# fanzhongyi/ExploreMultiModal

Hardware: AMD Instinct MI355X
Metric: image-text pairs/sec fwd+bwd, VLMo-Base, 1/2/4/8 MI355X; % bf16 MFMA roofline (higher is better)
Workload: dtype bf16

## Files before the change

exploremultimodal_amd/csrc/block.hip:

```cpp
#include "common.h"
#include "vlmo_hip.h"
#include <algorithm>
#include <map>
#include <vector>

namespace {
constexpr int GELU_DERIV = 4;


struct Events {
    std::vector<hipEvent_t> pool;
    hipEvent_t get(size_t i) {
        while (pool.size() <= i) {
            hipEvent_t e = nullptr;
            (void)hipEventCreateWithFlags(&e, hipEventDisableTiming);
            pool.push_back(e);
        }
        return pool[i];
    }
};
Events& events() {
    static thread_local std::map<int, Events> per_device;
    int dev = 0;
    (void)hipGetDevice(&dev);
// ... 288 lines not shown
    VLMO_CHECK_ARG(!two || nsets > batch || nb <= nsets,
                   "vlmo_stack_bwd: %d temporary sets cannot cover deferred batches of %d blocks", nsets, batch);
    Events& ev = events();
    Deferred D;
    D.store = s->wgrad_store != 0;
    std::vector<int> batch_of(nb, -1);
    int n_batches = 0, waited_upto = -1;
    auto flush = [&]() -> int {
        if (D.blocks.empty()) return 0;
        if (two) {
            hipEvent_t f = ev.get(2 * n_batches);
            (void)hipEventRecord(f, st);
            (void)hipStreamWaitEvent(side, f, 0);
        }
        std::stable_sort(D.tn.begin(), D.tn.end(), [](const VlmoTnProblem& a, const VlmoTnProblem& b) { return a.M > b.M; });
        TRY(vlmo_gemm_tn_multi(VLMO_BF16, D.tn.data(), (int)D.tn.size(), side));
        TRY(vlmo_colwork_multi(VLMO_BF16, D.col.data(), (int)D.col.size(), side));
        if (two) (void)hipEventRecord(ev.get(2 * n_batches + 1), side);
        if (s->grad_ready)
            for (int i : D.blocks)
                if (s->grad_ready[i]) (void)hipEventRecord((hipEvent_t)s->grad_ready[i], side);
        ++n_batches;
        D.tn.clear();
        D.col.clear();
        D.blocks.clear();
        return 0;
    };
    auto set_free = [&](int kk) -> int {
        if (!two || kk < nsets || kk >= nb) return 0;
        int need = batch_of[kk - nsets];
        if (need < 0 || need >= n_batches) {
            TRY(flush());
// ... 41 lines not shown
```

exploremultimodal_amd/csrc/elementwise.hip:

```cpp
#include "common.h"
#include "vlmo_hip.h"
#include <stdarg.h>
#include <stdio.h>

static thread_local char g_err[512] = "";
void vlmo_set_error(const char* fmt, ...) {
    va_list ap;
    va_start(ap, fmt);
    vsnprintf(g_err, sizeof(g_err), fmt, ap);
    va_end(ap);
}
extern "C" const char* vlmo_last_error(void) { return g_err; }
extern "C" int vlmo_abi_version(void) { return VLMO_ABI_VERSION; }

namespace {

__device__ __forceinline__ float fold_column(const float* __restrict__ ws, int ld, int ncols, int c, int r0, int r1) {
    float a = 0.f;
    if (c < ncols)
        for (int r = r0 + threadIdx.y; r < r1; r += 4) a += ws[(size_t)r * ld + c];
    return a;
}
template <typename T>
__device__ __forceinline__ void colsum8(const T* __restrict__ x, int ld, int ncols, int c8, int r0, int r1, float (&acc)[8]) {
    typedef typename Elem<T>::v8 v8;
#pragma unroll
    for (int j = 0; j < 8; ++j) acc[j] = 0.f;
    if (c8 < ncols) {
        for (int mb = r0 + threadIdx.y; mb < r1; mb += 16) {
            v8 v[4];
#pragma unroll
            for (int k = 0; k < 4; ++k) {
                const int m = mb + 4 * k;
                v[k] = *(const v8*)(x + (size_t)(m < r1 ? m : mb) * ld + c8);
            }
#pragma unroll
            for (int k = 0; k < 4; ++k)
                if (mb + 4 * k < r1)
#pragma unroll
                    for (int j = 0; j < 8; ++j) acc[j] += (float)v[k][j];
        }
    }
}

__global__ __launch_bounds__(256) void reduce_partials_kernel(const float* __restrict__ ws, int nblk, int ncols,
                                                              float* __restrict__ out0, int n0,
                                                              float* __restrict__ out1, int rows_per_slice,
                                                              float* __restrict__ out2, float* __restrict__ out3) {
    __shared__ float red[4][64];
    const int c = blockIdx.x * 64 + threadIdx.x;
    const int r0 = blockIdx.y * rows_per_slice, r1 = min(nblk, r0 + rows_per_slice);
    red[threadIdx.y][threadIdx.x] = fold_column(ws, ncols, ncols, c, r0, r1);
    __syncthreads();
    if (threadIdx.y == 0 && c < ncols) {
        const float t = red[0][threadIdx.x] + red[1][threadIdx.x] + red[2][threadIdx.x] + red[3][threadIdx.x];
        const int k = c / n0;
        float* base = k == 0 ? out0 : (k == 1 ? out1 : (k == 2 ? out2 : out3));
        if (base) atomicAdd(base + (c - k * n0), t);
    }
}

template <typename T> __device__ __forceinline__ f32x4 ld4(const T* p);
template <> __device__ __forceinline__ f32x4 ld4<bf16>(const bf16* p) {
    const bf16x4 v = *(const bf16x4*)p;
    return f32x4{(float)v[0], (float)v[1], (float)v[2], (float)v[3]};
}
template <> __device__ __forceinline__ f32x4 ld4<f16>(const f16* p) {
// ... 56 lines not shown
            ag += *(const f32x4*)(red + (y * 2 + 0) * d + c4);
            ab += *(const f32x4*)(red + (y * 2 + 1) * d + c4);
        }
        *(f32x4*)(ws + (size_t)blockIdx.x * 2 * d + c4) = ag;
        *(f32x4*)(ws + (size_t)blockIdx.x * 2 * d + d + c4) = ab;
    }
}

template <typename T>
__global__ __launch_bounds__(256) void colsum_kernel(const T* __restrict__ x, int ld, float* __restrict__ ws, int M,
                                                     int N, int rows_per_block) {
    __shared__ float red[4][64][8];
    const int c8 = (blockIdx.x * 64 + threadIdx.x) * 8;
    float acc[8];
    const int r0 = blockIdx.y * rows_per_block, r1 = min(M, r0 + rows_per_block);
    colsum8(x, ld, N, c8, r0, r1, acc);
#pragma unroll
    for (int j = 0; j < 8; ++j) red[threadIdx.y][threadIdx.x][j] = acc[j];
    __syncthreads();
    if (threadIdx.y == 0 && c8 < N) {
#pragma unroll
        for (int j = 0; j < 8; ++j)
            ws[(size_t)blockIdx.y * N + c8 + j] = red[0][threadIdx.x][j] + red[1][threadIdx.x][j] +
                                                  red[2][threadIdx.x][j] + red[3][threadIdx.x][j];
    }
}

constexpr int MAX_COL_JOBS = 32;
struct ColMulti {
    int n;
    int b0[MAX_COL_JOBS + 1];
    int gx[MAX_COL_JOBS], rps[MAX_COL_JOBS];
    VlmoColJob j[MAX_COL_JOBS];
};
template <typename T>
__global__ __launch_bounds__(256) void colwork_multi_kernel(const ColMulti cm) {
    __shared__ float red[4][64][8];
    int ji = 0;
#pragma unroll
    for (int q = 1; q < MAX_COL_JOBS; ++q)
        if (q < cm.n && (int)blockIdx.x >= cm.b0[q]) ji = q;
    ji = __builtin_amdgcn_readfirstlane(ji);
    const VlmoColJob& J = cm.j[ji];
    const int local = blockIdx.x - cm.b0[ji], gx = cm.gx[ji], rps = cm.rps[ji];
    const int bx = local % gx, by = local / gx;
    const int r0 = by * rps, r1 = min(J.rows, r0 + rps);
    const int tx = threadIdx.x, ty = threadIdx.y;
    if (J.kind == 0) {
        const int c = bx * 64 + tx;
        red[ty][tx][0] = fold_column((const float*)J.src, J.ld, J.ncols, c, r0, r1);
        __syncthreads();
        if (ty == 0 && c < J.ncols) {
            const float t = red[0][tx][0] + red[1][tx][0] + red[2][tx][0] + red[3][tx][0];
            const int k = c / J.n0;
            float* base = J.out[k];
            if (base) atomicAdd(base + (c - k * J.n0), t);
        }
    } else {
        const int c8 = (bx * 64 + tx) * 8;
        float acc[8];
        colsum8((const T*)J.src, J.ld, J.ncols, c8, r0, r1, acc);
#pragma unroll
        for (int jj = 0; jj < 8; ++jj) red[ty][tx][jj] = acc[jj];
        __syncthreads();
        if (ty == 0 && c8 < J.ncols) {
#pragma unroll
            for (int jj = 0; jj < 8; ++jj) {
                const int c = c8 + jj;
                const int k = c / J.n0;
                float* base = J.out[k];
                if (base) atomicAdd(base + (c - k * J.n0), red[0][tx][jj] + red[1][tx][jj] + red[2][tx][jj] + red[3][tx][jj]);
            }
        }
    }
}

template <typename T>
__global__ __launch_bounds__(256) void cast_weight_kernel(const float* __restrict__ src, int rows, int cols,
                                                          T* __restrict__ dst, T* __restrict__ dstT) {
    __shared__ float tile[32][33];
    const int c0 = blockIdx.x * 32, r0 = blockIdx.y * 32;
#pragma unroll
    for (int k = 0; k < 4; ++k) {
        const int r = r0 + threadIdx.y + 8 * k, c = c0 + threadIdx.x;
        float v = 0.f;
        if (r < rows && c < cols) {
            v = src[(size_t)r * cols + c];
            if (dst) dst[(size_t)r * cols + c] = (T)v;
        }
// ... 350 lines not shown
    for (int c = threadIdx.x; c < d; c += 256) {
        const int idx = embed_txt_red_index(c);
#pragma unroll
        for (int w = 0; w < 4; ++w) row[w * d + c] = red[0][w][idx] + red[1][w][idx] + red[2][w][idx] + red[3][w][idx];
    }
}

__global__ __launch_bounds__(256) void embed_txt_fold_kernel(const float* __restrict__ ws, int nrows, int maxlen, int d,
                                                             float* __restrict__ dln_w, float* __restrict__ dln_b,
                                                             float* __restrict__ dtype0, float* __restrict__ dbtype0,
                                                             float* __restrict__ dpos) {
    __shared__ float red[4][4][64];
    const int c = blockIdx.x * 64 + threadIdx.x, ld = 4 * d;
    if (blockIdx.y == 0) {
#pragma unroll
        for (int w = 0; w < 4; ++w) red[w][threadIdx.y][threadIdx.x] = fold_column(ws + w * d, ld, d, c, 0, nrows);
        __syncthreads();
        if (c < d) {
            const int w = threadIdx.y;
            float* out = w == 0 ? dln_w : (w == 1 ? dln_b : (w == 2 ? dtype0 : dbtype0));
            if (out) out[c] += red[w][0][threadIdx.x] + red[w][1][threadIdx.x] + red[w][2][threadIdx.x] + red[w][3][threadIdx.x];
        }
    } else {
        const int t = blockIdx.y - 1;
        red[0][threadIdx.y][threadIdx.x] = fold_column(ws + (size_t)t * ld + 3 * d, maxlen * ld, d, c, 0, nrows / maxlen);
        __syncthreads();
        if (threadIdx.y == 0 && c < d && dpos)
            dpos[(size_t)t * d + c] += red[0][0][threadIdx.x] + red[0][1][threadIdx.x] + red[0][2][threadIdx.x] + red[0][3][threadIdx.x];
    }
}

}

int fold_partials(const VlmoColJob& job, VlmoColJob* fold, hipStream_t stream) {
    if (fold) {
        *fold = job;
        return 0;
    }
    int slices = job.rows >= 64 ? 8 : 1;
    const int rps = (job.rows + slices - 1) / slices;
// ... 58 lines not shown
    if (dtype == VLMO_BF16)
        hipLaunchKernelGGL(colsum_kernel<bf16>, grid, block, 0, stream, (const bf16*)x, ld, ws, M, N, rpb);
    else if (dtype == VLMO_F16)
        hipLaunchKernelGGL(colsum_kernel<f16>, grid, block, 0, stream, (const f16*)x, ld, ws, M, N, rpb);
    else {
        vlmo_set_error("vlmo_colsum: dtype must be bf16 or f16");
        return -1;
    }
    VLMO_CHECK_LAUNCH("vlmo_colsum");
    return fold_partials(fold_job(ws, N, grid.y, N, N, out), nullptr, stream);
}

extern "C" int vlmo_colwork_multi(int dtype, const VlmoColJob* jobs, int n, hipStream_t stream) {
    VLMO_CHECK_ARG(jobs && n >= 1, "vlmo_colwork_multi: no jobs");
    VLMO_CHECK_ARG(dtype == VLMO_BF16 || dtype == VLMO_F16, "vlmo_colwork_multi: dtype must be bf16 or f16");
    for (int q0 = 0; q0 < n; q0 += MAX_COL_JOBS) {
        const int nq = n - q0 < MAX_COL_JOBS ? n - q0 : MAX_COL_JOBS;
        ColMulti cm{};
        cm.n = nq;
        int b = 0;
        for (int q = 0; q < nq; ++q) {
            const VlmoColJob& J = jobs[q0 + q];
            VLMO_CHECK_ARG(J.src && J.rows > 0 && J.ncols > 0 && J.n0 > 0 && J.ncols <= 4 * J.n0 && J.ld >= J.ncols,
                           "vlmo_colwork_multi: bad job %d", q0 + q);
            VLMO_CHECK_ARG(J.kind == 0 || (J.kind == 1 && J.ncols % 8 == 0 && J.ld % 8 == 0),
                           "vlmo_colwork_multi: job %d: matrix column sums need ncols, ld multiples of 8", q0 + q);
            cm.j[q] = J;
            cm.gx[q] = J.kind == 0 ? (J.ncols + 63) / 64 : (J.ncols / 8 + 63) / 64;
            int slices = J.kind == 0 ? (J.rows >= 64 ? 8 : 1) : (J.rows >= 2048 ? 32 : (J.rows >= 256 ? 8 : 1));
            int rps = (J.rows + slices - 1) / slices;
            if (J.kind == 1) rps = ((rps + 15) / 16) * 16;
            slices = (J.rows + rps - 1) / rps;
            cm.rps[q] = rps;
            cm.b0[q] = b;
            b += cm.gx[q] * slices;
        }
        for (int q = nq; q <= MAX_COL_JOBS; ++q) cm.b0[q] = b;
        if (dtype == VLMO_F16)
            hipLaunchKernelGGL(colwork_multi_kernel<f16>, dim3(b), dim3(64, 4), 0, stream, cm);
        else
            hipLaunchKernelGGL(colwork_multi_kernel<bf16>, dim3(b), dim3(64, 4), 0, stream, cm);
        VLMO_CHECK_LAUNCH("vlmo_colwork_multi");
    }
    return 0;
}

extern "C" int vlmo_cast_weight(int dtype, const float* src, int rows, int cols, void* dst, void* dstT,
                                hipStream_t stream) {
    VLMO_CHECK_ARG(src && (dst || dstT), "vlmo_cast_weight: null pointer");
    VLMO_CHECK_ARG(rows > 0 && cols > 0, "vlmo_cast_weight: empty matrix");
    dim3 grid((cols + 31) / 32, (rows + 31) / 32), block(32, 8);
    if (dtype == VLMO_BF16)
// ... 151 lines not shown
```

exploremultimodal_amd/csrc/gemm_tn.hip:

```cpp
#include "gemm_common.h"
#include "tn_multi_plan.h"

namespace {

struct GemmTN {
    const void* A;
    const void* B;
    float* C;
    int M, N1, N2, lda, ldb, ldc;
    int kt_per_split, tiles;
    float alpha;
    float* slab;
    int mode;
};

__device__ __attribute__((aligned(256))) char tn_zero_page[256];

__device__ __forceinline__ int tn_swz(int row) { return ((row & 3) << 2) | ((row >> 2) & 3); }

template <typename T, int BM, int BN, int WM, int WN, bool PP = false>
__device__ __forceinline__ void gemm_tn_body(const GemmTN& p, const int lid) {
    typedef typename Elem<T>::v8 v8;
    typedef typename Elem<T>::v4 v4;
    constexpr int NW = WM * WN;
// ... 227 lines not shown
                        atomicAdd(c, p.alpha * acc[i][j][r]);
                }
            }
        }
}

template <typename T, int BM, int BN, int WM, int WN, bool PP = false>
__global__ __launch_bounds__(WM * WN * 64, 2) void gemm_tn_kernel(const GemmTN p) {
    gemm_tn_body<T, BM, BN, WM, WN, PP>(p, xcd_remap(blockIdx.x, gridDim.x));
}
constexpr int TN_LDS_256 = 2 * 4 * 64 * 256;

struct GemmTNMulti {
    GemmTN p[MAX_TN_PROBS];
    uint16_t order[MAX_TN_ORDER];
};
template <typename T>
__global__ __launch_bounds__(512, 2) void gemm_tn_multi_kernel(const GemmTNMulti mp) {
    const uint32_t code = mp.order[blockIdx.x];
    if (code == TN_NOP) return;
    int gi = (int)(code >> 12);
    const int lid_in = __builtin_amdgcn_readfirstlane((int)(code & 0xFFFu));
    gi = __builtin_amdgcn_readfirstlane(gi);
    const GemmTN& q = mp.p[gi];
    GemmTN p;
    p.A = uniform_ptr(q.A), p.B = uniform_ptr(q.B), p.C = (float*)uniform_ptr(q.C);
    p.M = __builtin_amdgcn_readfirstlane(q.M), p.N1 = __builtin_amdgcn_readfirstlane(q.N1);
    p.N2 = __builtin_amdgcn_readfirstlane(q.N2), p.lda = __builtin_amdgcn_readfirstlane(q.lda);
    p.ldb = __builtin_amdgcn_readfirstlane(q.ldb), p.ldc = __builtin_amdgcn_readfirstlane(q.ldc);
    p.kt_per_split = __builtin_amdgcn_readfirstlane(q.kt_per_split), p.tiles = __builtin_amdgcn_readfirstlane(q.tiles);
    p.alpha = __builtin_bit_cast(float, __builtin_amdgcn_readfirstlane(__builtin_bit_cast(int, q.alpha)));
    p.slab = nullptr;
    p.mode = __builtin_amdgcn_readfirstlane(q.mode);
// ... 79 lines not shown
        if (dtype == VLMO_F16)
            hipLaunchKernelGGL((gemm_tn_kernel<f16, 128, 128, 2, 2>), grid, dim3(256), 65536, stream, p);
        else
            hipLaunchKernelGGL((gemm_tn_kernel<bf16, 128, 128, 2, 2>), grid, dim3(256), 65536, stream, p);
    }
    VLMO_CHECK_LAUNCH("vlmo_gemm_tn");
    if (use_slab) {
        const long total = (long)N1 * (N2 / 4);
        const int rg = (int)((total + 255) / 256 < 2048 ? (total + 255) / 256 : 2048);
        hipLaunchKernelGGL(tn_reduce_kernel, dim3(rg), dim3(256), 0, stream, ws, pl.splits, N1, N2, C, ldc, alpha);
        VLMO_CHECK_LAUNCH("vlmo_gemm_tn(reduce)");
    }
    return 0;
}

extern "C" int vlmo_gemm_tn_multi(int dtype, const VlmoTnProblem* probs, int n, hipStream_t stream) {
    VLMO_CHECK_ARG(probs && n >= 1, "vlmo_gemm_tn_multi: no problems");
    VLMO_CHECK_ARG(dtype == VLMO_BF16 || dtype == VLMO_F16, "vlmo_gemm_tn_multi: dtype must be bf16 or f16");
    for (int q = 0; q < n; ++q) {
        const VlmoTnProblem& r = probs[q];
        VLMO_CHECK_ARG(r.A && r.B && r.C, "vlmo_gemm_tn_multi: null operand in problem %d", q);
        VLMO_CHECK_ARG(r.M > 0 && r.N1 >= 8 && r.N2 >= 8 && r.N1 % 8 == 0 && r.N2 % 8 == 0 && r.lda % 8 == 0 &&
                           r.ldb % 8 == 0 && r.lda >= r.N1 && r.ldb >= r.N2 && r.ldc >= r.N2,
                       "vlmo_gemm_tn_multi: bad shape in problem %d (M=%d N1=%d N2=%d)", q, r.M, r.N1, r.N2);
    }
    const TnMultiPlan plan = plan_tn_multi(probs, n);
    VLMO_CHECK_ARG(plan.error.empty(), "%s", plan.error.c_str());
    static DeviceOnce attr;
    if (attr.first()) {
        (void)hipFuncSetAttribute((const void*)gemm_tn_multi_kernel<bf16>, hipFuncAttributeMaxDynamicSharedMemorySize, TN_LDS_256);
        (void)hipFuncSetAttribute((const void*)gemm_tn_multi_kernel<f16>, hipFuncAttributeMaxDynamicSharedMemorySize, TN_LDS_256);
    }
    for (const TnLaunchPlan& L : plan.launches) {
        GemmTNMulti mp{};
        double flops = 0;
        for (int q = 0; q < L.nq; ++q) {
            const VlmoTnProblem& r = probs[L.q0 + q];
            const VlmoTnProblemPlan& s = L.p[q];
            if (s.zero_first) {
                hipError_t rc = hipMemset2DAsync(r.C, (size_t)r.ldc * 4, 0, (size_t)r.N2 * 4, r.N1, stream);
                if (rc != hipSuccess) {
                    vlmo_set_error("vlmo_gemm_tn_multi: memset failed: %s", hipGetErrorString(rc));
                    return (int)rc;
                }
            }
            mp.p[q] = GemmTN{r.A, r.B, r.C, r.M, r.N1, r.N2, r.lda, r.ldb, r.ldc, s.kt_per_split, s.tiles, r.alpha, nullptr, s.mode};
            flops += 2.0 * r.M * r.N1 * r.N2;
        }
        std::copy(L.order, L.order + L.grid, mp.order);
        ProfScope prof(73, flops, stream);
        if (dtype == VLMO_F16)
            hipLaunchKernelGGL((gemm_tn_multi_kernel<f16>), dim3(L.grid), dim3(512), TN_LDS_256, stream, mp);
        else
            hipLaunchKernelGGL((gemm_tn_multi_kernel<bf16>), dim3(L.grid), dim3(512), TN_LDS_256, stream, mp);
        VLMO_CHECK_LAUNCH("vlmo_gemm_tn_multi");
    }
    return 0;
}

extern "C" int vlmo_gemm_tn_multi_plan(const VlmoTnProblem* probs, int n, int32_t* n_launches, int32_t* launch_q0,
                                       VlmoTnProblemPlan* prob, int32_t* grid, uint16_t* order) {
    VLMO_CHECK_ARG(probs && n >= 1, "vlmo_gemm_tn_multi: no problems");
    VLMO_CHECK_ARG(n_launches && launch_q0 && prob && grid && order, "vlmo_gemm_tn_multi_plan: null output");
    const TnMultiPlan plan = plan_tn_multi(probs, n);
    VLMO_CHECK_ARG(plan.error.empty(), "%s", plan.error.c_str());
    *n_launches = (int32_t)plan.launches.size();
    for (size_t k = 0; k < plan.launches.size(); ++k) {
        const TnLaunchPlan& L = plan.launches[k];
        launch_q0[k] = L.q0, launch_q0[k + 1] = L.q0 + L.nq;
        std::copy(L.p, L.p + L.nq, prob + L.q0);
        grid[k] = L.grid;
        std::copy(L.order, L.order + L.grid, order + k * MAX_TN_ORDER);
    }
    return 0;
}
```

exploremultimodal_amd/csrc/tn_multi_plan.h:

```cpp
#pragma once
#include "vlmo_hip.h"
#include <algorithm>
#include <cstdio>
#include <string>
#include <vector>

constexpr int MAX_TN_PROBS = 16;
constexpr int MAX_TN_ORDER = 1024;
constexpr uint16_t TN_NOP = 0xFFFF;
enum { TN_ATOMIC = 0, TN_ACCUM = 1, TN_STORE = 2 };

struct TnLaunchPlan {
    int q0, nq;
    VlmoTnProblemPlan p[MAX_TN_PROBS];
    int grid;
    uint16_t order[MAX_TN_ORDER];
};
struct TnMultiPlan {
    std::vector<TnLaunchPlan> launches;
    std::string error;
};

inline int64_t tn_tiles256(const VlmoTnProblem& r) { return (((int64_t)r.N1 + 255) / 256) * (((int64_t)r.N2 + 255) / 256); }
inline int tn_ktiles(const VlmoTnProblem& r) { return (int)(((int64_t)r.M + 63) / 64); }
// ... 47 lines not shown
            for (int x = 0; x < 8; ++x)
                for (size_t k = i + cnt * x / 8; k < i + cnt * (x + 1) / 8; ++k) bins[x].push_back(jobs[k].code);
        }
        size_t deepest = 0;
        for (int x = 0; x < 8; ++x) deepest = std::max(deepest, bins[x].size());
        if (deepest * 8 > (size_t)MAX_TN_ORDER)
            return fail("vlmo_gemm_tn_multi: %zu workgroups exceed one launch (pass fewer problems per call)", jobs.size());
        L.grid = (int)deepest * 8;
        for (int b = 0; b < L.grid; ++b) {
            const std::vector<uint16_t>& bin = bins[b & 7];
            L.order[b] = (size_t)(b >> 3) < bin.size() ? bin[b >> 3] : TN_NOP;
        }
    }
    return plan;
}
```

exploremultimodal_amd/hip.py:

```python
import ctypes
import os

import numpy as np
import torch

_HERE = os.path.dirname(os.path.abspath(__file__))
LIB_PATH = os.environ.get('VLMO_HIP_LIB') or os.path.join(_HERE, 'lib', 'libvlmo_hip.so')

BF16, F16, F32 = 0, 1, 2
EPI_BIAS, EPI_BIAS_GELU, EPI_RESID, EPI_DGELU, EPI_F32, EPI_DUAL, EPI_ARGMAX, EPI_CE, EPI_CE_BWD = 0, 1, 2, 3, 4, 5, 6, 7, 8

_vp, _i32, _u32, _u64, _f32, _i64 = (ctypes.c_void_p, ctypes.c_int32, ctypes.c_uint32,
                                     ctypes.c_uint64, ctypes.c_float, ctypes.c_int64)


class Epilogue(ctypes.Structure):
    _fields_ = [('out', _vp), ('out2', _vp), ('bias', _vp), ('gamma', _vp),
                ('resid', _vp), ('row_scale', _vp), ('row_index', _vp), ('aux', _vp),
                ('ldo', _i32), ('ld2', _i32), ('relu', _i32),
                ('drop_thresh', _u32), ('inv_keep', _f32), ('beta', _f32),
                ('seed', _u64), ('colpart', _vp)]


_fp = _vp
# ... 87 lines not shown
    'vlmo_argmax_reduce': [_vp, _i32, _vp, _i32, _vp],
    'vlmo_dvae_embed': [_vp, _vp, _vp, _vp, _i32, _i32, _i32, _vp],
    'vlmo_upsample2_nhwc': [_vp, _vp, _i32, _i32, _i32, _i32, _vp],
    'vlmo_dvae_out_head': [_vp, _vp, _vp, _vp, _i32, _i32, _i32, _i32, _i32, _vp],
    'vlmo_conv4s2_nhwc': [_i32, _vp, _i32, _i32, _i32, _i32, _vp, _i32, _vp, ctypes.POINTER(Epilogue), _vp],
    'vlmo_convt4s2_nhwc': [_i32, _vp, _i32, _i32, _i32, _i32, _vp, _i32, _vp, ctypes.POINTER(Epilogue), _vp],
    'vlmo_dvae_patch4s2': [_vp, _vp, _i32, _i32, _i32, _i32, _i32, _vp],
    'vlmo_dvae_out_head_linear': [_vp, _vp, _vp, _vp, _i32, _i32, _i32, _i32, _i32, _vp],
    'vlmo_ce_reduce': [_vp, _i32, _vp, _i32, _vp, _vp, _vp, _i32, _vp],
    'vlmo_stack_fwd': [ctypes.POINTER(StackDesc), _vp],
    'vlmo_stack_bwd': [ctypes.POINTER(StackDesc), _vp],
    'vlmo_gemm_tn_multi': [_i32, ctypes.POINTER(TnProblem), _i32, _vp],
    'vlmo_gemm_tn_multi_plan': [ctypes.POINTER(TnProblem), _i32, ctypes.POINTER(_i32), ctypes.POINTER(_i32),
                                ctypes.POINTER(TnProblemPlan), ctypes.POINTER(_i32), ctypes.POINTER(ctypes.c_uint16)],
    'vlmo_colwork_multi': [_i32, ctypes.POINTER(ColJob), _i32, _vp],
    'vlmo_event_create': [ctypes.POINTER(ctypes.c_void_p)],
    'vlmo_event_destroy': [_vp],
    'vlmo_stream_wait_event': [_vp, _vp],
    'vlmo_profile_start': [_i32],
    'vlmo_gemm_nt_grouped': [_i32, _i32, _i32, _i32, _vp, _i32, _vp, _i32, _vp, _i32, _i32, _vp, _vp],
    'vlmo_mt_grad_norm': [ctypes.c_void_p, _f32, _f32, _vp, _vp, _vp],
    'vlmo_mt_adam': [ctypes.c_void_p, ctypes.c_void_p, _vp, _vp],
    'vlmo_mt_ema': [ctypes.c_void_p, _f32, _vp],
    'vlmo_mt_adam_ema': [ctypes.c_void_p, ctypes.c_void_p, _vp, _vp, _f32, _vp],
    'vlmo_side_stream_create': [_i32, ctypes.POINTER(ctypes.c_uint32), _i32, ctypes.POINTER(ctypes.c_void_p)],
    'vlmo_profile_stop': [_i32, ctypes.POINTER(ctypes.c_double), ctypes.POINTER(ctypes.c_double),
                          ctypes.POINTER(ctypes.c_int64)],
    'vlmo_gemm_nt_2src': [_i32, _i32, _i32, _vp, _i32, _i32, _f32, _vp, _i32, _vp, _i32, _i32, _i32, _i32,
                          ctypes.POINTER(Epilogue), _vp],
    'vlmo_comm_available': [],
# ... 8 lines not shown
    'vlmo_grad_unpack': [_vp, _vp, _i64, _vp],
    'vlmo_ln_gelu_fwd': [_vp, _i32, _vp, _vp, _vp, _i32, _vp, _vp, _i32, _i32, _f32, _vp],
    'vlmo_ln_gelu_bwd': [_vp, _i32, _vp, _i32, _vp, _vp, _vp, _vp, _vp, _i32, _vp, _i32, _vp, _vp, _vp, _i32, _i32, _vp,
                         _i64, _vp],
    'vlmo_vqa_bce': [_vp, _i32, _vp, _i32, _i32, _i32, _vp, _vp, _vp, _vp, _f32, _vp, _i32, _vp, _i32, _vp],
    'vlmo_isda_update': [_vp, _i32, _vp, _vp, _vp, _vp, _vp, _i32, _i32, _i32, _i32, _vp, _vp, _vp, _vp, _vp],
    'vlmo_isda_aug_fwd': [_vp, _i32, _vp, _vp, _i32, _i32, _i32, _i32, _f32, _vp, _i32, _vp, _i64, _vp],
    'vlmo_isda_aug_bwd': [_vp, _i32, _vp, _i32, _vp, _vp, _i32, _i32, _i32, _i32, _f32, _vp, _i32, _vp, _i64, _vp],
    'vlmo_sim_topk': [_vp, _i32, _vp, _i32, _i32, _i32, _i32, _i32, _f32, _i32, _vp, ctypes.c_size_t, _vp, _vp, _vp],
    'vlmo_crop_resample': [_vp, _i64, _vp, _vp, _i32, _vp, _vp, _i32, ctypes.POINTER(_f32), ctypes.POINTER(_f32), _f32, _vp,
                           _i64, _vp],
    'vlmo_randaug': [_vp, _vp, _vp, _i64, _vp, _vp, _i32, _vp, _vp, _i32, _i32, _vp, _i64, _vp],
}

_lib = None
ABI_VERSION = 16

def lib():
    global _lib
    if _lib is None:
        if not os.path.exists(LIB_PATH):
            raise RuntimeError(
                f'{LIB_PATH} not found: build the HIP extension first '
                '(python -c "import __graft_entry__ as g; g.build()" or '
                'make -C exploremultimodal_amd/csrc). There is no CPU fallback.')
        L = ctypes.CDLL(LIB_PATH)
        L.vlmo_last_error.restype = ctypes.c_char_p
        L.vlmo_abi_version.restype = ctypes.c_int
        if L.vlmo_abi_version() != ABI_VERSION:
            raise RuntimeError(f'{LIB_PATH} has ABI version {L.vlmo_abi_version()}, this package needs {ABI_VERSION}: '
                               'rebuild it (make -C exploremultimodal_amd/csrc)')
# ... 319 lines not shown
                                  _stream())
    _check(rc, 'vlmo_convt4s2_nhwc')


def dvae_patch4s2(x, out, Kpad):
    B, C, H, W = x.shape
    _check(lib().vlmo_dvae_patch4s2(_p(x), _p(out), B, C, H, W, Kpad, _stream()), 'vlmo_dvae_patch4s2')


def dvae_out_head_linear(x, w, bias, out, B, H, W):
    Cout, C = w.shape
    _check(lib().vlmo_dvae_out_head_linear(_p(x), _p(w), _p(bias), _p(out), B, H, W, C, Cout, _stream()),
           'vlmo_dvae_out_head_linear')


def gemm_tn_multi(problems, dtype=BF16):
    n = len(problems)
    arr = (TnProblem * n)()
    for i, (A, B, C, M, N1, N2, acc, *alpha) in enumerate(problems):
        arr[i] = TnProblem(_p(A), _p(B), _p(C), A.stride(0), B.stride(0), C.stride(0), M, N1, N2,
                           float(alpha[0]) if alpha else 1.0, int(acc))
    _check(lib().vlmo_gemm_tn_multi(dtype, arr, n, _stream()), 'vlmo_gemm_tn_multi')


TN_ORDER, TN_NOP = 1024, 0xFFFF


def gemm_tn_multi_plan(shapes):
    n = len(shapes)
    arr = (TnProblem * n)()
    for i, (M, N1, N2, acc) in enumerate(shapes):
        arr[i] = TnProblem(None, None, None, N1, N2, N2, M, N1, N2, 1.0, int(acc))
    nl, q0 = _i32(0), (_i32 * (n + 1))()
    pp, grid, order = (TnProblemPlan * n)(), (_i32 * n)(), (ctypes.c_uint16 * (n * TN_ORDER))()
    _check(lib().vlmo_gemm_tn_multi_plan(arr, n, ctypes.byref(nl), q0, pp, grid, order), 'vlmo_gemm_tn_multi_plan')
    return [dict(q0=q0[k], nq=q0[k + 1] - q0[k],
                 problems=[(p.tiles, p.splits, p.kt_per_split, p.mode, p.zero_first) for p in pp[q0[k]:q0[k + 1]]],
                 grid=grid[k], order=list(order[k * TN_ORDER:k * TN_ORDER + grid[k]]))
            for k in range(nl.value)]


def colwork_multi(jobs, dtype=BF16):
    n = len(jobs)
    arr = (ColJob * n)()
    for i, (kind, src, rows, ncols, outs, n0) in enumerate(jobs):
        o = (ctypes.c_void_p * 4)(*[_p(t) for t in (list(outs) + [None] * 4)[:4]])
        arr[i] = ColJob(kind, src.stride(0), _p(src), rows, ncols, o, n0, 0)
    _check(lib().vlmo_colwork_multi(dtype, arr, n, _stream()), 'vlmo_colwork_multi')


def event_create():
    out = ctypes.c_void_p()
    _check(lib().vlmo_event_create(ctypes.byref(out)), 'vlmo_event_create')
    return out.value


def stream_wait_event(stream, ev):
    raw = stream.cuda_stream if hasattr(stream, 'cuda_stream') else stream
    _check(lib().vlmo_stream_wait_event(raw, ev), 'vlmo_stream_wait_event')


COMM_ID_BYTES = 128

# ... 279 lines not shown
```

include/vlmo_hip.h:

```cpp
#ifndef VLMO_HIP_H
#define VLMO_HIP_H

#include <stddef.h>
#include <stdint.h>

#ifdef __cplusplus
extern "C" {
#endif

#ifndef __HIP_PLATFORM_AMD__
typedef struct ihipStream_t* hipStream_t;
#endif

enum { VLMO_BF16 = 0, VLMO_F16 = 1, VLMO_F32 = 2 };

enum {
    VLMO_EPI_BIAS = 0,
    VLMO_EPI_BIAS_GELU = 1,
    VLMO_EPI_RESID = 2,
    VLMO_EPI_DGELU = 3,
    VLMO_EPI_F32 = 4,
    VLMO_EPI_DUAL = 5,
    VLMO_EPI_ARGMAX = 6,
    VLMO_EPI_CE = 7,
// ... 7 lines not shown
    const float* gamma;
    const float* resid;
    const float* row_scale;
    const int32_t* row_index;
    const void* aux;
    int32_t ldo, ld2;
    int32_t relu;
    uint32_t drop_thresh;
    float inv_keep;
    float beta;
    uint64_t seed;
    float* colpart;
} VlmoEpilogue;

const char* vlmo_last_error(void);
#define VLMO_ABI_VERSION 16
int vlmo_abi_version(void);

int vlmo_gemm_nt(int epi, int dtype, int tile, const void* A, int lda, const void* B, int ldb,
                 int M, int N, int K, const VlmoEpilogue* e, hipStream_t stream);
int vlmo_gemm_nt_2src(int epi, int dtype, int tile, const void* A, int lda, int k1, float seg_scale, const void* A2,
                      int lda2, const void* B, int ldb, int M, int N, int K, const VlmoEpilogue* e,
                      hipStream_t stream);
int vlmo_gemm_nt_grouped(int epi, int dtype, int tile, int ngroups, const void* const* A, int lda,
                         const void* const* B, int ldb, const int32_t* M, int N, int K,
                         const VlmoEpilogue* e, hipStream_t stream);

int64_t vlmo_gemm_tn_ws_bytes(int M, int N1, int N2);
int vlmo_gemm_tn(int dtype, const void* A, int lda, const void* B, int ldb, float* C, int ldc,
                 int M, int N1, int N2, float alpha, int splits, float* ws, int64_t ws_bytes,
                 hipStream_t stream);
// ... 56 lines not shown
                   const int32_t* row_index, void* dz, float* dgamma, float* dbias, int M, int d,
                   uint32_t drop_thresh,
                   float inv_keep, uint64_t seed, float* ws, int64_t ws_bytes, hipStream_t stream);

int vlmo_colsum(int dtype, const void* x, int ld, float* out, int M, int N, float* ws,
                int64_t ws_bytes, hipStream_t stream);

typedef struct VlmoColJob {
    int32_t kind, ld;
    const void* src;
    int32_t rows, ncols;
    float* out[4];
    int32_t n0, pad_;
} VlmoColJob;
int vlmo_colwork_multi(int dtype, const VlmoColJob* jobs, int n, hipStream_t stream);

int vlmo_cast_weight(int dtype, const float* src, int rows, int cols, void* dst, void* dstT,
                     hipStream_t stream);
int vlmo_cast_weight_multi(int dtype, int n, const float* const* src, const int32_t* rows, const int32_t* cols,
                           void* const* dst, void* const* dstT, hipStream_t stream);

int vlmo_patchify(const float* img, void* out, int B, int C, int H, int W, int patch,
                  hipStream_t stream);
int vlmo_embed_img_finish(const void* proj, const float* cls_tok, const float* mask_tok,
                          const float* pos, const float* type_row, const uint8_t* masked_pos,
                          float* x, int B, int npatch, int d, uint32_t drop_thresh,
                          float inv_keep, uint64_t seed, hipStream_t stream);
int vlmo_embed_img_bwd(const float* dx, const uint8_t* masked_pos, void* dproj, float* dcls,
                       float* dmask, float* dpos, float* dtype_row, int B, int npatch, int d,
                       uint32_t drop_thresh, float inv_keep, uint64_t seed, hipStream_t stream);
// ... 222 lines not shown
```

Baseline: 4513.

## Fuse column-reduction jobs into the TN weight-gradient GEMM launch tail

Column-sum jobs (bias/gamma gradients) now run inside the last grouped TN GEMM launch instead of a separate kernel. Extra workgroups are appended to fill the partial last wave across 256 CUs, or 32 extra when the wave is full. Those workgroups loop over the column units with an 8-row-lane reduction. This removes one kernel launch and uses idle CUs in the GEMM tail, but the reduction blocks run under the GEMM kernel's launch bounds and LDS allocation and could contend with GEMM tiles.

```diff
diff --git a/exploremultimodal_amd/csrc/block.hip b/exploremultimodal_amd/csrc/block.hip
--- a/exploremultimodal_amd/csrc/block.hip
+++ b/exploremultimodal_amd/csrc/block.hip
@@ -326,8 +326,7 @@
             (void)hipStreamWaitEvent(side, f, 0);
         }
         std::stable_sort(D.tn.begin(), D.tn.end(), [](const VlmoTnProblem& a, const VlmoTnProblem& b) { return a.M > b.M; });
-        TRY(vlmo_gemm_tn_multi(VLMO_BF16, D.tn.data(), (int)D.tn.size(), side));
-        TRY(vlmo_colwork_multi(VLMO_BF16, D.col.data(), (int)D.col.size(), side));
+        TRY(vlmo_gemm_tn_multi_cols(VLMO_BF16, D.tn.data(), (int)D.tn.size(), D.col.data(), (int)D.col.size(), side));
         if (two) (void)hipEventRecord(ev.get(2 * n_batches + 1), side);
         if (s->grad_ready)
             for (int i : D.blocks)
diff --git a/exploremultimodal_amd/csrc/colwork.h b/exploremultimodal_amd/csrc/colwork.h
--- /dev/null
+++ b/exploremultimodal_amd/csrc/colwork.h
@@ -0,0 +1,132 @@
+#pragma once
+#include "common.h"
+
+constexpr int MAX_COL_JOBS = 32;
+struct ColMulti {
+    int n;
+    int b0[MAX_COL_JOBS + 1];
+    int gx[MAX_COL_JOBS], rps[MAX_COL_JOBS];
+    VlmoColJob j[MAX_COL_JOBS];
+};
+
+inline int check_col_jobs(const char* who, const VlmoColJob* jobs, int n) {
+    for (int q = 0; q < n; ++q) {
+        const VlmoColJob& J = jobs[q];
+        VLMO_CHECK_ARG(J.src && J.rows > 0 && J.ncols > 0 && J.n0 > 0 && J.ncols <= 4 * J.n0 && J.ld >= J.ncols,
+                       "%s: bad job %d", who, q);
+        VLMO_CHECK_ARG(J.kind == 0 || (J.kind == 1 && J.ncols % 8 == 0 && J.ld % 8 == 0),
+                       "%s: job %d: matrix column sums need ncols, ld multiples of 8", who, q);
+    }
+    return 0;
+}
+inline int col_multi_fill(const VlmoColJob* jobs, int nq, ColMulti& cm) {
+    cm.n = nq;
+    int b = 0;
+    for (int q = 0; q < nq; ++q) {
+        const VlmoColJob& J = jobs[q];
+        cm.j[q] = J;
+        cm.gx[q] = J.kind == 0 ? (J.ncols + 63) / 64 : (J.ncols / 8 + 63) / 64;
+        int slices = J.kind == 0 ? (J.rows >= 64 ? 8 : 1) : (J.rows >= 2048 ? 32 : (J.rows >= 256 ? 8 : 1));
+        int rps = (J.rows + slices - 1) / slices;
+        if (J.kind == 1) rps = ((rps + 15) / 16) * 16;
+        slices = (J.rows + rps - 1) / rps;
+        cm.rps[q] = rps;
+        cm.b0[q] = b;
+        b += cm.gx[q] * slices;
+    }
+    for (int q = nq; q <= MAX_COL_JOBS; ++q) cm.b0[q] = b;
+    return b;
+}
+
+template <int NY = 4, int U = 1>
+__device__ __forceinline__ float fold_column(const float* __restrict__ ws, int ld, int ncols, int c, int r0, int r1, int ty) {
+    float a = 0.f;
+    if (c < ncols)
+        for (int r = r0 + ty; r < r1; r += U * NY) {
+            float v[U];
+#pragma unroll
+            for (int k = 0; k < U; ++k) {
+                const int m = r + k * NY;
+                v[k] = ws[(size_t)(m < r1 ? m : r) * ld + c];
+            }
+#pragma unroll
+            for (int k = 0; k < U; ++k)
+                a += r + k * NY < r1 ? v[k] : 0.f;
+        }
+    return a;
+}
+template <typename T, int NY = 4>
+__device__ __forceinline__ void colsum8(const T* __restrict__ x, int ld, int ncols, int c8, int r0, int r1, int ty, float (&acc)[8]) {
+    typedef typename Elem<T>::v8 v8;
+#pragma unroll
+    for (int j = 0; j < 8; ++j) acc[j] = 0.f;
+    if (c8 < ncols) {
+        for (int mb = r0 + ty; mb < r1; mb += 4 * NY) {
+            v8 v[4];
+#pragma unroll
+            for (int k = 0; k < 4; ++k) {
+                const int m = mb + NY * k;
+                v[k] = *(const v8*)(x + (size_t)(m < r1 ? m : mb) * ld + c8);
+            }
+#pragma unroll
+            for (int k = 0; k < 4; ++k)
+                if (mb + NY * k < r1)
+#pragma unroll
+                    for (int j = 0; j < 8; ++j) acc[j] += (float)v[k][j];
+        }
+    }
+}
+
+template <int NY, int K>
+__device__ __forceinline__ void col_lanes_to_red(float (&a)[K], int tx, int ty, float (*red)[64][8]) {
+    static_assert(NY == 4 || NY == 8, "four or eight row lanes");
+    if constexpr (NY == 8) {
+        if (ty >= 4)
+#pragma unroll
+            for (int j = 0; j < K; ++j) red[ty - 4][tx][j] = a[j];
+        __syncthreads();
+        if (ty < 4)
+#pragma unroll
+            for (int j = 0; j < K; ++j) a[j] += red[ty][tx][j];
+    }
+    if (NY == 4 || ty < 4)
+#pragma unroll
+        for (int j = 0; j < K; ++j) red[ty][tx][j] = a[j];
+    __syncthreads();
+}
+__device__ __forceinline__ void col_add_out(const VlmoColJob& J, int c, float t) {
+    const int k = c / J.n0;
+    float* base = J.out[k];
+    if (base) atomicAdd(base + (c - k * J.n0), t);
+}
+
+__device__ __forceinline__ int col_job_of(const ColMulti& cm, int unit) {
+    int ji = 0;
+#pragma unroll
+    for (int q = 1; q < MAX_COL_JOBS; ++q)
+        if (q < cm.n && unit >= cm.b0[q]) ji = q;
+    return __builtin_amdgcn_readfirstlane(ji);
+}
+template <typename T, int NY>
+__device__ __forceinline__ void col_unit(const ColMulti& cm, int ji, int unit, int tx, int ty, float (*red)[64][8]) {
+    const VlmoColJob& J = cm.j[ji];
+    const int local = unit - cm.b0[ji], gx = cm.gx[ji], rps = cm.rps[ji];
+    const int bx = local % gx, by = local / gx;
+    const int r0 = by * rps, r1 = min(J.rows, r0 + rps);
+    if (J.kind == 0) {
+        const int c = bx * 64 + tx;
+        float a[1] = {fold_column<NY, NY == 8 ? 4 : 1>((const float*)J.src, J.ld, J.ncols, c, r0, r1, ty)};
+        col_lanes_to_red<NY>(a, tx, ty, red);
+        if (ty == 0 && c < J.ncols) col_add_out(J, c, red[0][tx][0] + red[1][tx][0] + red[2][tx][0] + red[3][tx][0]);
+    } else {
+        const int c8 = (bx * 64 + tx) * 8;
+        float acc[8];
+        colsum8<T, NY>((const T*)J.src, J.ld, J.ncols, c8, r0, r1, ty, acc);
+        col_lanes_to_red<NY>(acc, tx, ty, red);
+        if (ty == 0 && c8 < J.ncols) {
+#pragma unroll
+            for (int jj = 0; jj < 8; ++jj)
+                col_add_out(J, c8 + jj, red[0][tx][jj] + red[1][tx][jj] + red[2][tx][jj] + red[3][tx][jj]);
+        }
+    }
+}
diff --git a/exploremultimodal_amd/csrc/elementwise.hip b/exploremultimodal_amd/csrc/elementwise.hip
--- a/exploremultimodal_amd/csrc/elementwise.hip
+++ b/exploremultimodal_amd/csrc/elementwise.hip
@@ -1,4 +1,4 @@
-#include "common.h"
+#include "colwork.h"
 #include "vlmo_hip.h"
 #include <stdarg.h>
 #include <stdio.h>
@@ -15,33 +15,6 @@
 
 namespace {
 
-__device__ __forceinline__ float fold_column(const float* __restrict__ ws, int ld, int ncols, int c, int r0, int r1) {
-    float a = 0.f;
-    if (c < ncols)
-        for (int r = r0 + threadIdx.y; r < r1; r += 4) a += ws[(size_t)r * ld + c];
-    return a;
-}
-template <typename T>
-__device__ __forceinline__ void colsum8(const T* __restrict__ x, int ld, int ncols, int c8, int r0, int r1, float (&acc)[8]) {
-    typedef typename Elem<T>::v8 v8;
-#pragma unroll
-    for (int j = 0; j < 8; ++j) acc[j] = 0.f;
-    if (c8 < ncols) {
-        for (int mb = r0 + threadIdx.y; mb < r1; mb += 16) {
-            v8 v[4];
-#pragma unroll
-            for (int k = 0; k < 4; ++k) {
-                const int m = mb + 4 * k;
-                v[k] = *(const v8*)(x + (size_t)(m < r1 ? m : mb) * ld + c8);
-            }
-#pragma unroll
-            for (int k = 0; k < 4; ++k)
-                if (mb + 4 * k < r1)
-#pragma unroll
-                    for (int j = 0; j < 8; ++j) acc[j] += (float)v[k][j];
-        }
-    }
-}
 
 __global__ __launch_bounds__(256) void reduce_partials_kernel(const float* __restrict__ ws, int nblk, int ncols,
                                                               float* __restrict__ out0, int n0,
@@ -50,7 +23,7 @@
     __shared__ float red[4][64];
     const int c = blockIdx.x * 64 + threadIdx.x;
     const int r0 = blockIdx.y * rows_per_slice, r1 = min(nblk, r0 + rows_per_slice);
-    red[threadIdx.y][threadIdx.x] = fold_column(ws, ncols, ncols, c, r0, r1);
+    red[threadIdx.y][threadIdx.x] = fold_column(ws, ncols, ncols, c, r0, r1, threadIdx.y);
     __syncthreads();
     if (threadIdx.y == 0 && c < ncols) {
         const float t = red[0][threadIdx.x] + red[1][threadIdx.x] + red[2][threadIdx.x] + red[3][threadIdx.x];
@@ -137,7 +110,7 @@
     const int c8 = (blockIdx.x * 64 + threadIdx.x) * 8;
     float acc[8];
     const int r0 = blockIdx.y * rows_per_block, r1 = min(M, r0 + rows_per_block);
-    colsum8(x, ld, N, c8, r0, r1, acc);
+    colsum8(x, ld, N, c8, r0, r1, threadIdx.y, acc);
 #pragma unroll
     for (int j = 0; j < 8; ++j) red[threadIdx.y][threadIdx.x][j] = acc[j];
     __syncthreads();
@@ -149,53 +122,10 @@
     }
 }
 
-constexpr int MAX_COL_JOBS = 32;
-struct ColMulti {
-    int n;
-    int b0[MAX_COL_JOBS + 1];
-    int gx[MAX_COL_JOBS], rps[MAX_COL_JOBS];
-    VlmoColJob j[MAX_COL_JOBS];
-};
 template <typename T>
 __global__ __launch_bounds__(256) void colwork_multi_kernel(const ColMulti cm) {
     __shared__ float red[4][64][8];
-    int ji = 0;
-#pragma unroll
-    for (int q = 1; q < MAX_COL_JOBS; ++q)
-        if (q < cm.n && (int)blockIdx.x >= cm.b0[q]) ji = q;
-    ji = __builtin_amdgcn_readfirstlane(ji);
-    const VlmoColJob& J = cm.j[ji];
-    const int local = blockIdx.x - cm.b0[ji], gx = cm.gx[ji], rps = cm.rps[ji];
-    const int bx = local % gx, by = local / gx;
-    const int r0 = by * rps, r1 = min(J.rows, r0 + rps);
-    const int tx = threadIdx.x, ty = threadIdx.y;
-    if (J.kind == 0) {
-        const int c = bx * 64 + tx;
-        red[ty][tx][0] = fold_column((const float*)J.src, J.ld, J.ncols, c, r0, r1);
-        __syncthreads();
-        if (ty == 0 && c < J.ncols) {
-            const float t = red[0][tx][0] + red[1][tx][0] + red[2][tx][0] + red[3][tx][0];
-            const int k = c / J.n0;
-            float* base = J.out[k];
-            if (base) atomicAdd(base + (c - k * J.n0), t);
-        }
-    } else {
-        const int c8 = (bx * 64 + tx) * 8;
-        float acc[8];
-        colsum8((const T*)J.src, J.ld, J.ncols, c8, r0, r1, acc);
-#pragma unroll
-        for (int jj = 0; jj < 8; ++jj) red[ty][tx][jj] = acc[jj];
-        __syncthreads();
-        if (ty == 0 && c8 < J.ncols) {
-#pragma unroll
-            for (int jj = 0; jj < 8; ++jj) {
-                const int c = c8 + jj;
-                const int k = c / J.n0;
-                float* base = J.out[k];
-                if (base) atomicAdd(base + (c - k * J.n0), red[0][tx][jj] + red[1][tx][jj] + red[2][tx][jj] + red[3][tx][jj]);
-            }
-        }
-    }
+    col_unit<T, 4>(cm, col_job_of(cm, blockIdx.x), blockIdx.x, threadIdx.x, threadIdx.y, red);
 }
 
 template <typename T>
@@ -576,7 +506,7 @@
     const int c = blockIdx.x * 64 + threadIdx.x, ld = 4 * d;
     if (blockIdx.y == 0) {
 #pragma unroll
-        for (int w = 0; w < 4; ++w) red[w][threadIdx.y][threadIdx.x] = fold_column(ws + w * d, ld, d, c, 0, nrows);
+        for (int w = 0; w < 4; ++w) red[w][threadIdx.y][threadIdx.x] = fold_column(ws + w * d, ld, d, c, 0, nrows, threadIdx.y);
         __syncthreads();
         if (c < d) {
             const int w = threadIdx.y;
@@ -585,7 +515,7 @@
         }
     } else {
         const int t = blockIdx.y - 1;
-        red[0][threadIdx.y][threadIdx.x] = fold_column(ws + (size_t)t * ld + 3 * d, maxlen * ld, d, c, 0, nrows / maxlen);
+        red[0][threadIdx.y][threadIdx.x] = fold_column(ws + (size_t)t * ld + 3 * d, maxlen * ld, d, c, 0, nrows / maxlen, threadIdx.y);
         __syncthreads();
         if (threadIdx.y == 0 && c < d && dpos)
             dpos[(size_t)t * d + c] += red[0][0][threadIdx.x] + red[0][1][threadIdx.x] + red[0][2][threadIdx.x] + red[0][3][threadIdx.x];
@@ -674,28 +604,10 @@
 extern "C" int vlmo_colwork_multi(int dtype, const VlmoColJob* jobs, int n, hipStream_t stream) {
     VLMO_CHECK_ARG(jobs && n >= 1, "vlmo_colwork_multi: no jobs");
     VLMO_CHECK_ARG(dtype == VLMO_BF16 || dtype == VLMO_F16, "vlmo_colwork_multi: dtype must be bf16 or f16");
+    if (int rc = check_col_jobs("vlmo_colwork_multi", jobs, n)) return rc;
     for (int q0 = 0; q0 < n; q0 += MAX_COL_JOBS) {
-        const int nq = n - q0 < MAX_COL_JOBS ? n - q0 : MAX_COL_JOBS;
         ColMulti cm{};
-        cm.n = nq;
-        int b = 0;
-        for (int q = 0; q < nq; ++q) {
-            const VlmoColJob& J = jobs[q0 + q];
-            VLMO_CHECK_ARG(J.src && J.rows > 0 && J.ncols > 0 && J.n0 > 0 && J.ncols <= 4 * J.n0 && J.ld >= J.ncols,
-                           "vlmo_colwork_multi: bad job %d", q0 + q);
-            VLMO_CHECK_ARG(J.kind == 0 || (J.kind == 1 && J.ncols % 8 == 0 && J.ld % 8 == 0),
-                           "vlmo_colwork_multi: job %d: matrix column sums need ncols, ld multiples of 8", q0 + q);
-            cm.j[q] = J;
-            cm.gx[q] = J.kind == 0 ? (J.ncols + 63) / 64 : (J.ncols / 8 + 63) / 64;
-            int slices = J.kind == 0 ? (J.rows >= 64 ? 8 : 1) : (J.rows >= 2048 ? 32 : (J.rows >= 256 ? 8 : 1));
-            int rps = (J.rows + slices - 1) / slices;
-            if (J.kind == 1) rps = ((rps + 15) / 16) * 16;
-            slices = (J.rows + rps - 1) / rps;
-            cm.rps[q] = rps;
-            cm.b0[q] = b;
-            b += cm.gx[q] * slices;
-        }
-        for (int q = nq; q <= MAX_COL_JOBS; ++q) cm.b0[q] = b;
+        const int b = col_multi_fill(jobs + q0, n - q0 < MAX_COL_JOBS ? n - q0 : MAX_COL_JOBS, cm);
         if (dtype == VLMO_F16)
             hipLaunchKernelGGL(colwork_multi_kernel<f16>, dim3(b), dim3(64, 4), 0, stream, cm);
         else
diff --git a/exploremultimodal_amd/csrc/gemm_tn.hip b/exploremultimodal_amd/csrc/gemm_tn.hip
--- a/exploremultimodal_amd/csrc/gemm_tn.hip
+++ b/exploremultimodal_amd/csrc/gemm_tn.hip
@@ -1,4 +1,5 @@
 #include "gemm_common.h"
+#include "colwork.h"
 #include "tn_multi_plan.h"
 
 namespace {
@@ -265,9 +266,22 @@
 struct GemmTNMulti {
     GemmTN p[MAX_TN_PROBS];
     uint16_t order[MAX_TN_ORDER];
+    int grid;
 };
 template <typename T>
-__global__ __launch_bounds__(512, 2) void gemm_tn_multi_kernel(const GemmTNMulti mp) {
+__global__ __launch_bounds__(512, 2) void gemm_tn_multi_kernel(const GemmTNMulti mp, const ColMulti cm) {
+    if ((int)blockIdx.x >= mp.grid) {
+        extern __shared__ __attribute__((aligned(16))) char smem[];
+        float(*red)[64][8] = (float(*)[64][8])smem;
+        const int tx = threadIdx.x & 63, ty = __builtin_amdgcn_readfirstlane(threadIdx.x >> 6);
+        const int ncw = gridDim.x - mp.grid, units = cm.b0[MAX_COL_JOBS];
+        for (int u = blockIdx.x - mp.grid, ji = 0; u < units; u += ncw) {
+            while (u >= cm.b0[ji + 1]) ++ji;
+            col_unit<T, 8>(cm, ji, u, tx, ty, red);
+            __syncthreads();
+        }
+        return;
+    }
     const uint32_t code = mp.order[blockIdx.x];
     if (code == TN_NOP) return;
     int gi = (int)(code >> 12);
@@ -377,16 +391,18 @@
     return 0;
 }
 
-extern "C" int vlmo_gemm_tn_multi(int dtype, const VlmoTnProblem* probs, int n, hipStream_t stream) {
-    VLMO_CHECK_ARG(probs && n >= 1, "vlmo_gemm_tn_multi: no problems");
-    VLMO_CHECK_ARG(dtype == VLMO_BF16 || dtype == VLMO_F16, "vlmo_gemm_tn_multi: dtype must be bf16 or f16");
+namespace {
+int tn_multi_run(const char* who, int dtype, const VlmoTnProblem* probs, int n, const VlmoColJob* jobs, int nj,
+                 hipStream_t stream) {
+    VLMO_CHECK_ARG(dtype == VLMO_BF16 || dtype == VLMO_F16, "%s: dtype must be bf16 or f16", who);
     for (int q = 0; q < n; ++q) {
         const VlmoTnProblem& r = probs[q];
-        VLMO_CHECK_ARG(r.A && r.B && r.C, "vlmo_gemm_tn_multi: null operand in problem %d", q);
+        VLMO_CHECK_ARG(r.A && r.B && r.C, "%s: null operand in problem %d", who, q);
         VLMO_CHECK_ARG(r.M > 0 && r.N1 >= 8 && r.N2 >= 8 && r.N1 % 8 == 0 && r.N2 % 8 == 0 && r.lda % 8 == 0 &&
                            r.ldb % 8 == 0 && r.lda >= r.N1 && r.ldb >= r.N2 && r.ldc >= r.N2,
-                       "vlmo_gemm_tn_multi: bad shape in problem %d (M=%d N1=%d N2=%d)", q, r.M, r.N1, r.N2);
-    }
+                       "%s: bad shape in problem %d (M=%d N1=%d N2=%d)", who, q, r.M, r.N1, r.N2);
+    }
+    if (int rc = check_col_jobs(who, jobs, nj)) return rc;
     const TnMultiPlan plan = plan_tn_multi(probs, n);
     VLMO_CHECK_ARG(plan.error.empty(), "%s", plan.error.c_str());
     static DeviceOnce attr;
@@ -394,8 +410,17 @@
         (void)hipFuncSetAttribute((const void*)gemm_tn_multi_kernel<bf16>, hipFuncAttributeMaxDynamicSharedMemorySize, TN_LDS_256);
         (void)hipFuncSetAttribute((const void*)gemm_tn_multi_kernel<f16>, hipFuncAttributeMaxDynamicSharedMemorySize, TN_LDS_256);
     }
+    const int ride = std::min(nj, MAX_COL_JOBS);
+    if (nj > ride)
+        if (int rc = vlmo_colwork_multi(dtype, jobs, nj - ride, stream)) return rc;
     for (const TnLaunchPlan& L : plan.launches) {
         GemmTNMulti mp{};
+        ColMulti cm{};
+        int ncw = 0;
+        if (ride && &L == &plan.launches.back()) {
+            col_multi_fill(jobs + (nj - ride), ride, cm);
+            ncw = tn_col_workgroups(L.grid);
+        }
         double flops = 0;
         for (int q = 0; q < L.nq; ++q) {
             const VlmoTnProblem& r = probs[L.q0 + q];
@@ -403,7 +428,7 @@
             if (s.zero_first) {
                 hipError_t rc = hipMemset2DAsync(r.C, (size_t)r.ldc * 4, 0, (size_t)r.N2 * 4, r.N1, stream);
                 if (rc != hipSuccess) {
-                    vlmo_set_error("vlmo_gemm_tn_multi: memset failed: %s", hipGetErrorString(rc));
+                    vlmo_set_error("%s: memset failed: %s", who, hipGetErrorString(rc));
                     return (int)rc;
                 }
             }
@@ -411,14 +436,29 @@
             flops += 2.0 * r.M * r.N1 * r.N2;
         }
         std::copy(L.order, L.order + L.grid, mp.order);
+        mp.grid = L.grid;
         ProfScope prof(73, flops, stream);
         if (dtype == VLMO_F16)
-            hipLaunchKernelGGL((gemm_tn_multi_kernel<f16>), dim3(L.grid), dim3(512), TN_LDS_256, stream, mp);
+            hipLaunchKernelGGL((gemm_tn_multi_kernel<f16>), dim3(L.grid + ncw), dim3(512), TN_LDS_256, stream, mp, cm);
         else
-            hipLaunchKernelGGL((gemm_tn_multi_kernel<bf16>), dim3(L.grid), dim3(512), TN_LDS_256, stream, mp);
-        VLMO_CHECK_LAUNCH("vlmo_gemm_tn_multi");
+            hipLaunchKernelGGL((gemm_tn_multi_kernel<bf16>), dim3(L.grid + ncw), dim3(512), TN_LDS_256, stream, mp, cm);
+        VLMO_CHECK_LAUNCH(who);
     }
     return 0;
+}
+}
+
+extern "C" int vlmo_gemm_tn_multi(int dtype, const VlmoTnProblem* probs, int n, hipStream_t stream) {
+    VLMO_CHECK_ARG(probs && n >= 1, "vlmo_gemm_tn_multi: no problems");
+    return tn_multi_run("vlmo_gemm_tn_multi", dtype, probs, n, nullptr, 0, stream);
+}
+
+extern "C" int vlmo_gemm_tn_multi_cols(int dtype, const VlmoTnProblem* probs, int n, const VlmoColJob* jobs, int ncols_jobs,
+                                       hipStream_t stream) {
+    VLMO_CHECK_ARG(n >= 0 && ncols_jobs >= 0 && (probs || n == 0) && (jobs || ncols_jobs == 0) && n + ncols_jobs >= 1,
+                   "vlmo_gemm_tn_multi_cols: no problems and no jobs");
+    if (n == 0) return vlmo_colwork_multi(dtype, jobs, ncols_jobs, stream);
+    return tn_multi_run("vlmo_gemm_tn_multi_cols", dtype, probs, n, jobs, ncols_jobs, stream);
 }
 
 extern "C" int vlmo_gemm_tn_multi_plan(const VlmoTnProblem* probs, int n, int32_t* n_launches, int32_t* launch_q0,
@@ -437,3 +477,28 @@
     }
     return 0;
 }
+
+extern "C" int vlmo_gemm_tn_multi_cols_plan(const VlmoTnProblem* probs, int n, const VlmoColJob* jobs, int ncols_jobs,
+                                            int32_t* grid, int32_t* ncw, int32_t* first_job, int32_t* n_units,
+                                            int32_t* units, int32_t cap) {
+    VLMO_CHECK_ARG(probs && n >= 1 && jobs && ncols_jobs >= 1, "vlmo_gemm_tn_multi_cols_plan: no problems or no jobs");
+    VLMO_CHECK_ARG(grid && ncw && first_job && n_units && (units || cap <= 0), "vlmo_gemm_tn_multi_cols_plan: null output");
+    for (int q = 0; q < ncols_jobs; ++q)
+        VLMO_CHECK_ARG((jobs[q].kind == 0 || jobs[q].kind == 1) && jobs[q].rows > 0 && jobs[q].ncols > 0,
+                       "vlmo_gemm_tn_multi_cols_plan: bad job %d", q);
+    const TnMultiPlan plan = plan_tn_multi(probs, n);
+    VLMO_CHECK_ARG(plan.error.empty(), "%s", plan.error.c_str());
+    const int ride = std::min(ncols_jobs, MAX_COL_JOBS);
+    ColMulti cm{};
+    *n_units = col_multi_fill(jobs + (ncols_jobs - ride), ride, cm);
+    *first_job = ncols_jobs - ride;
+    *grid = plan.launches.back().grid;
+    *ncw = tn_col_workgroups(*grid);
+    for (int u = 0, q = 0; u < *n_units && u < cap; ++u) {
+        while (u >= cm.b0[q + 1]) ++q;
+        const int local = u - cm.b0[q];
+        units[4 * u] = *first_job + q, units[4 * u + 1] = local % cm.gx[q], units[4 * u + 2] = local / cm.gx[q];
+        units[4 * u + 3] = tn_col_unit_workgroup(*grid, *ncw, u);
+    }
+    return 0;
+}
diff --git a/exploremultimodal_amd/csrc/tn_multi_plan.h b/exploremultimodal_amd/csrc/tn_multi_plan.h
--- a/exploremultimodal_amd/csrc/tn_multi_plan.h
+++ b/exploremultimodal_amd/csrc/tn_multi_plan.h
@@ -85,3 +85,11 @@
     }
     return plan;
 }
+
+constexpr int TN_CUS = 256;
+constexpr int TN_COL_WGS_FULL = 32;
+inline int tn_col_workgroups(int grid) {
+    const int rem = grid % TN_CUS;
+    return rem ? TN_CUS - rem : TN_COL_WGS_FULL;
+}
+inline int tn_col_unit_workgroup(int grid, int ncw, int u) { return grid + u % ncw; }
diff --git a/exploremultimodal_amd/hip.py b/exploremultimodal_amd/hip.py
--- a/exploremultimodal_amd/hip.py
+++ b/exploremultimodal_amd/hip.py
@@ -125,6 +125,9 @@
     'vlmo_gemm_tn_multi_plan': [ctypes.POINTER(TnProblem), _i32, ctypes.POINTER(_i32), ctypes.POINTER(_i32),
                                 ctypes.POINTER(TnProblemPlan), ctypes.POINTER(_i32), ctypes.POINTER(ctypes.c_uint16)],
     'vlmo_colwork_multi': [_i32, ctypes.POINTER(ColJob), _i32, _vp],
+    'vlmo_gemm_tn_multi_cols': [_i32, ctypes.POINTER(TnProblem), _i32, ctypes.POINTER(ColJob), _i32, _vp],
+    'vlmo_gemm_tn_multi_cols_plan': [ctypes.POINTER(TnProblem), _i32, ctypes.POINTER(ColJob), _i32] +
+                                    [ctypes.POINTER(_i32)] * 5 + [_i32],
     'vlmo_event_create': [ctypes.POINTER(ctypes.c_void_p)],
     'vlmo_event_destroy': [_vp],
     'vlmo_stream_wait_event': [_vp, _vp],
@@ -163,7 +166,7 @@
 }
 
 _lib = None
-ABI_VERSION = 16
+ABI_VERSION = 17
 
 def lib():
     global _lib
@@ -513,13 +516,29 @@
            'vlmo_dvae_out_head_linear')
 
 
-def gemm_tn_multi(problems, dtype=BF16):
-    n = len(problems)
-    arr = (TnProblem * n)()
+def _tn_problems(problems):
+    arr = (TnProblem * max(1, len(problems)))()
     for i, (A, B, C, M, N1, N2, acc, *alpha) in enumerate(problems):
         arr[i] = TnProblem(_p(A), _p(B), _p(C), A.stride(0), B.stride(0), C.stride(0), M, N1, N2,
                            float(alpha[0]) if alpha else 1.0, int(acc))
-    _check(lib().vlmo_gemm_tn_multi(dtype, arr, n, _stream()), 'vlmo_gemm_tn_multi')
+    return arr
+
+
+def _col_jobs(jobs):
+    arr = (ColJob * max(1, len(jobs)))()
+    for i, (kind, src, rows, ncols, outs, n0) in enumerate(jobs):
+        o = (ctypes.c_void_p * 4)(*[_p(t) for t in (list(outs) + [None] * 4)[:4]])
+        arr[i] = ColJob(kind, src.stride(0), _p(src), rows, ncols, o, n0, 0)
+    return arr
+
+
+def gemm_tn_multi(problems, dtype=BF16):
+    _check(lib().vlmo_gemm_tn_multi(dtype, _tn_problems(problems), len(problems), _stream()), 'vlmo_gemm_tn_multi')
+
+
+def gemm_tn_multi_cols(problems, jobs, dtype=BF16):
+    _check(lib().vlmo_gemm_tn_multi_cols(dtype, _tn_problems(problems), len(problems), _col_jobs(jobs), len(jobs),
+                                         _stream()), 'vlmo_gemm_tn_multi_cols')
 
 
 TN_ORDER, TN_NOP = 1024, 0xFFFF
@@ -539,13 +558,25 @@
             for k in range(nl.value)]
 
 
+def gemm_tn_multi_cols_plan(shapes, jobs):
+    n, nj = len(shapes), len(jobs)
+    arr = (TnProblem * n)()
+    for i, (M, N1, N2, acc) in enumerate(shapes):
+        arr[i] = TnProblem(None, None, None, N1, N2, N2, M, N1, N2, 1.0, int(acc))
+    cj = (ColJob * nj)()
+    for i, (kind, rows, ncols) in enumerate(jobs):
+        cj[i] = ColJob(kind, ncols, None, rows, ncols, (ctypes.c_void_p * 4)(), ncols, 0)
+    grid, ncw, first, nu = _i32(0), _i32(0), _i32(0), _i32(0)
+    out = [ctypes.byref(v) for v in (grid, ncw, first, nu)]
+    _check(lib().vlmo_gemm_tn_multi_cols_plan(arr, n, cj, nj, *out, None, 0), 'vlmo_gemm_tn_multi_cols_plan')
+    units = (_i32 * (4 * nu.value))()
+    _check(lib().vlmo_gemm_tn_multi_cols_plan(arr, n, cj, nj, *out, units, nu.value), 'vlmo_gemm_tn_multi_cols_plan')
+    return dict(grid=grid.value, ncw=ncw.value, first_job=first.value,
+                units=[tuple(units[4 * u:4 * u + 4]) for u in range(nu.value)])
+
+
 def colwork_multi(jobs, dtype=BF16):
-    n = len(jobs)
-    arr = (ColJob * n)()
-    for i, (kind, src, rows, ncols, outs, n0) in enumerate(jobs):
-        o = (ctypes.c_void_p * 4)(*[_p(t) for t in (list(outs) + [None] * 4)[:4]])
-        arr[i] = ColJob(kind, src.stride(0), _p(src), rows, ncols, o, n0, 0)
-    _check(lib().vlmo_colwork_multi(dtype, arr, n, _stream()), 'vlmo_colwork_multi')
+    _check(lib().vlmo_colwork_multi(dtype, _col_jobs(jobs), len(jobs), _stream()), 'vlmo_colwork_multi')
 
 
 def event_create():
diff --git a/include/vlmo_hip.h b/include/vlmo_hip.h
--- a/include/vlmo_hip.h
+++ b/include/vlmo_hip.h
@@ -45,7 +45,7 @@
 } VlmoEpilogue;
 
 const char* vlmo_last_error(void);
-#define VLMO_ABI_VERSION 16
+#define VLMO_ABI_VERSION 17
 int vlmo_abi_version(void);
 
 int vlmo_gemm_nt(int epi, int dtype, int tile, const void* A, int lda, const void* B, int ldb,
@@ -132,6 +132,12 @@
     int32_t n0, pad_;
 } VlmoColJob;
 int vlmo_colwork_multi(int dtype, const VlmoColJob* jobs, int n, hipStream_t stream);
+
+int vlmo_gemm_tn_multi_cols(int dtype, const VlmoTnProblem* probs, int n, const VlmoColJob* jobs, int ncols_jobs,
+                            hipStream_t stream);
+int vlmo_gemm_tn_multi_cols_plan(const VlmoTnProblem* probs, int n, const VlmoColJob* jobs, int ncols_jobs,
+                                 int32_t* grid, int32_t* ncw, int32_t* first_job, int32_t* n_units, int32_t* units,
+                                 int32_t cap);
 
 int vlmo_cast_weight(int dtype, const float* src, int rows, int cols, void* dst, void* dstT,
                      hipStream_t stream);
```

Result: no change. 4542, median of 6 (+0.6%).
